# hasindu2008/squigulator

Hardware: AMD Instinct MI355X
Metric: simulated raw samples/sec (higher is better)
Workload: dtype f32+f64

## Files before the change

### squigulator_amd/csrc/h_common.h

```cpp
#pragma once

#if defined(SQG_DEV)
#define SQG_DEV_ENV(name) getenv(name)
#else
#define SQG_DEV_ENV(name) (static_cast<const char*>(nullptr))
#endif
static inline int dev_env_int(const char* v, int dflt) { return v ? atoi(v) : dflt; }

#ifndef SQG_SOURCE_HASH
#define SQG_SOURCE_HASH "unstamped"
#endif
extern "C" const char sqg_source_hash_marker[] = "SQG_SOURCE_HASH=" SQG_SOURCE_HASH ";";
#if defined(SQG_DEV)
static const char kBuildInfo[] = "source_hash=" SQG_SOURCE_HASH ";dev=1";
#else
static const char kBuildInfo[] = "source_hash=" SQG_SOURCE_HASH ";dev=0";
#endif
extern "C" const char* sqg_build_info(void) { return kBuildInfo; }

#include "h_cpus.h"

static uint32_t lcg_pow(uint32_t base, unsigned long long e) {
    uint32_t r = 1, b = base;
    while (e) { if (e & 1) r = lcg_mul(r, b); b = lcg_mul(b, b); e >>= 1; }
// ... 124 lines not shown
    HostPool pool_threads;
    struct DrawAhead* draw_ahead = nullptr;
    sqg_cfg_t cfg;
    int k = 0, num_kmer = 0, T = 0, wlo = 0, whi = 0, nw = 0;
    hipStream_t stream = nullptr;
    uint32_t* d_rows = nullptr;
    float2* d_model = nullptr;
    uint32_t* d_pow = nullptr;
    std::vector<uint32_t> h_pow;
    uint32_t jump2(unsigned long long n) const {
        if (n >> 32) return lcg_pow(lcg_mul(LCG_A, LCG_A), n);
        uint32_t r = h_pow[2 * POW_N + (size_t)(n & (POW_N - 1))];
        const uint32_t hi = (uint32_t)(n >> 10) & (POW_N - 1), hi2 = (uint32_t)(n >> 20);
        if (hi) r = lcg_mul(r, h_pow[3 * POW_N + hi]);
        if (hi2) r = lcg_mul(r, h_pow[4 * POW_N + hi2]);
        return r;
    }
    unsigned int* d_err = nullptr;
    unsigned long long fix_tickets = 0;
    unsigned long long scan_tickets = 0;
    struct Slot {
        int16_t* d_sig = nullptr; size_t sig_cap = 0;
        long long* d_sigoff = nullptr; size_t reads_cap = 0;
        FixEntry* d_fix = nullptr; size_t fix_cap = 0;
        unsigned int* d_fix_count = nullptr;
        FixEntry* d_fix_sh = nullptr; size_t fix_sh_cap = 0;
        unsigned int fix_sh_per = 0;
        unsigned int* d_fix_sh_count = nullptr;
        uint2* d_evrec = nullptr; size_t evrec_cap = 0;
        int* d_slow = nullptr; size_t slow_cap = 0;
        ItemDesc* d_items = nullptr; size_t items_cap = 0;
        uint32_t* d_part = nullptr; size_t part_cap = 0;
        uint32_t* d_lbase = nullptr; size_t lbase_cap = 0;
        int* d_tile_link = nullptr; size_t tile_link_cap = 0;
        uint32_t* d_part_state = nullptr; size_t part_state_cap = 0;
        hipEvent_t cal_a = nullptr, cal_b = nullptr; bool cal_pending = false; long long cal_events = 0; int cal_tries = 0; float cal_ps = 0.f;
        uint2* cal_prev = nullptr; float cal_prev_ps = 0.f;
        unsigned long long gen = 0;
        hipEvent_t done = nullptr;
        hipEvent_t sampled = nullptr;
    } slot[2];
    struct CountSet {
        uint16_t* d_dwell = nullptr; size_t dwell_cap = 0;
        uint32_t* d_tile_so = nullptr; size_t tile_cap = 0;
        unsigned long long* d_seglen = nullptr; size_t seglen_cap = 0;
        size_t seglen_dirty = 0;
        unsigned long long gen = 0;
    } cset[3];
    int num_cu = 256;
    std::deque<sqg_batch*> staged_q;
    hipStream_t fix_stream = nullptr;
    unsigned long long* d_scan_part = nullptr; size_t scan_part_cap = 0;
    uint32_t* d_link_rows = nullptr; size_t link_rows_cap = 0;
    uint32_t* d_pcnt[2] = {nullptr, nullptr}; size_t pcnt_cap[2] = {0, 0};
    uint32_t* d_slice = nullptr; size_t slice_cap = 0;
    uint32_t* d_phist = nullptr; size_t phist_cap = 0;
    double row_bound = 0;
    bool range_mode = false;
    uint32_t* d_xcounts = nullptr; size_t xcounts_cap = 0;
    struct Recycled { uint8_t* d_block; size_t block_bytes; long long* h_sigoff; long long* h_sigoff_dev; size_t h_n; hipEvent_t ev[8];
                      uint8_t* h_meta; size_t h_meta_bytes; hipEvent_t ev_staged; };
    std::vector<Recycled> pool;
    hipStream_t stage_stream = nullptr;
    std::vector<uint32_t> time_c;
    std::vector<long long> off_x, med_x;
    unsigned long long next_stage = 0, next_run = 0, compress_seq = 0;
    unsigned long long runs = 0;
    unsigned int* d_mid_done = nullptr;
    int stage_threads = 0;
    int stage_threads_last = 0;
    int phase_timing_every = 1;
    std::set<unsigned long long> abandoned;
    sqg_timing_t timing = {0, 0, 0, 0, 0, 0, 0, 0};
    bool use_dwell_stream = true, use_kmer_streams = true;
    float delta_x = 0.f;
    float delta_x_measured = 0.f;
    double amp_floor = 0, amp_ceil = 0;
// ... 276 lines not shown
```

### squigulator_amd/csrc/h_context.h

```cpp
#pragma once

extern "C" const char* sqg_strerror(int code) {
    switch (code) {
    case SQG_OK: return "ok";
    case SQG_EINVAL: return "invalid argument or unsupported configuration";
    case SQG_ENOMEM: return "out of memory";
    case SQG_EDEVICE: return "HIP runtime error";
    case SQG_ESEQUENCE: return "batches must be run in staging order";
    case SQG_ENODEVICE: return "no usable HIP device";
    case SQG_EOVERFLOW: return "read too long (>= UINT32_MAX samples) or dwell > 65535";
    case SQG_EIO: return "file I/O error";
    default: return "unknown error";
    }
}

extern "C" const char* sqg_last_error(const sqg_ctx_t* ctx) { return ctx ? ctx->err.c_str() : ""; }

extern "C" int sqg_device_count(void) {
    int n = 0;
    if (hipGetDeviceCount(&n) != hipSuccess) return SQG_ENODEVICE;
    return n;
}

extern "C" int32_t sqg_worker_of(int32_t i, int32_t n_rec, int32_t T) {
    if (T <= 1 || n_rec <= 0) return 0;
    const int32_t step = (n_rec + T - 1) / T;
    return i / step;
}

extern "C" void sqg_destroy(sqg_ctx_t* ctx) {
    if (!ctx) return;
    if (ctx->b5_reader_drain) ctx->b5_reader_drain(ctx->b5_reader, true);
    (void)hipSetDevice(ctx->cfg.device);
    if (ctx->b5_stream) { (void)hipStreamSynchronize(ctx->b5_stream); (void)hipStreamDestroy(ctx->b5_stream); ctx->b5_stream = nullptr; }
    if (ctx->stream) (void)hipStreamSynchronize(ctx->stream);
    if (ctx->fix_stream) (void)hipStreamSynchronize(ctx->fix_stream);
    delete ctx->draw_ahead; ctx->draw_ahead = nullptr;
    (void)hipFree(ctx->d_pcnt[0]); (void)hipFree(ctx->d_pcnt[1]); (void)hipFree(ctx->d_slice); (void)hipFree(ctx->d_phist);
    (void)hipFree(ctx->d_rows); (void)hipFree(ctx->d_link_rows); (void)hipFree(ctx->d_scan_part); (void)hipFree(ctx->d_xcounts); (void)hipFree(ctx->d_model); (void)hipFree(ctx->d_samp_scratch); (void)hipFree(ctx->d_pow); (void)hipFree(ctx->d_err); (void)hipFree(ctx->d_mid_done); if (ctx->h_samp) (void)hipHostFree(ctx->h_samp);
    for (auto& Q : ctx->cset) { (void)hipFree(Q.d_dwell); (void)hipFree(Q.d_tile_so); (void)hipFree(Q.d_seglen); }
    for (auto& S : ctx->slot) {
        (void)hipFree(S.d_sig); (void)hipFree(S.d_sigoff);
        (void)hipFree(S.d_fix); (void)hipFree(S.d_fix_count); (void)hipFree(S.d_fix_sh); (void)hipFree(S.d_fix_sh_count);
        (void)hipFree(S.d_evrec); (void)hipFree(S.d_slow);
        (void)hipFree(S.d_items); (void)hipFree(S.d_part_state); (void)hipFree(S.d_part); (void)hipFree(S.d_lbase); (void)hipFree(S.d_tile_link);
        (void)hipFree(S.cal_prev);
        if (S.cal_a) (void)hipEventDestroy(S.cal_a);
        if (S.cal_b) (void)hipEventDestroy(S.cal_b);
        if (S.done) (void)hipEventDestroy(S.done);
        if (S.sampled) (void)hipEventDestroy(S.sampled);
    }
    (void)hipFree(ctx->d_svb); (void)hipFree(ctx->d_svb_size); (void)hipFree(ctx->d_svb_off);
    (void)hipFree(ctx->d_b5meta); (void)hipFree(ctx->d_b5out); (void)hipFree(ctx->d_b5tab); (void)hipFree(ctx->d_b5size); for (auto* q : ctx->h_b5out) if (q) (void)hipHostFree(q); if (ctx->h_b5meta) (void)hipHostFree(ctx->h_b5meta);
    ctx->chunk.release();
    ctx->site.release();
    ctx->event.release();
    ctx->pileup.release();
    ctx->detect.release();
    ctx->align.release();
    ctx->collapse.release();
    ctx->scale.release();
    (void)hipFree(ctx->d_genome); (void)hipFree(ctx->d_contig_off); (void)hipFree(ctx->d_cum); (void)hipFree(ctx->d_nprefix);
    (void)hipFree(ctx->d_trans_csum); (void)hipFree(ctx->d_trans_idx); (void)hipFree(ctx->d_samp);
    (void)hipFree(ctx->d_meth); (void)hipFree(ctx->d_meth_has); (void)hipFree(ctx->d_meth_st);
    if (ctx->stage_stream) { (void)hipStreamSynchronize(ctx->stage_stream); (void)hipStreamDestroy(ctx->stage_stream); }
    for (auto& r : ctx->pool) { (void)hipFree(r.d_block); (void)hipHostFree(r.h_sigoff); (void)hipHostFree(r.h_meta); for (auto& e : r.ev) if (e) (void)hipEventDestroy(e); if (r.ev_staged) (void)hipEventDestroy(r.ev_staged); }
    ctx->pool.clear();
    if (ctx->fix_stream) (void)hipStreamDestroy(ctx->fix_stream);
    if (ctx->stream) (void)hipStreamDestroy(ctx->stream);
    delete ctx;
}

extern "C" int sqg_create(const sqg_cfg_t* cfg, sqg_ctx_t** out) {
    if (!cfg || !out) return SQG_EINVAL;
    *out = nullptr;
    if (cfg->abi_version != SQG_ABI_VERSION) return SQG_EINVAL;
    if (cfg->kmer_size < 1 || cfg->kmer_size > 9 || !cfg->model) return SQG_EINVAL;
    if (cfg->num_workers < 1 || cfg->worker_lo < 0 || cfg->worker_hi > cfg->num_workers || cfg->worker_lo >= cfg->worker_hi) return SQG_EINVAL;
// ... 162 lines not shown
```

### squigulator_amd/csrc/h_run.h

```cpp
#pragma once

static void count_params(sqg_ctx* c, const sqg_batch* b, sqg_ctx::CountSet& Q, const int n_part, uint32_t* d_pcnt, SigParams& P) {
    const sqg_profile_t& p = c->cfg.profile;
    P.reads = b->d_reads; P.chain_off = b->d_chain_off; P.chain_reads = b->d_chain_reads; P.chain_order = b->d_chain_order; P.bases = b->d_bases;
    P.dwell = c->use_dwell_stream ? Q.d_dwell : nullptr; P.dwell_out = Q.d_dwell; P.seglen_out = Q.d_seglen; P.seglen = Q.d_seglen; P.tile_so = Q.d_tile_so;
    P.dmean = p.dwell_mean; P.dstd = p.dwell_std; P.pw = c->d_pow; P.err = b->d_err; P.delta_x = c->delta_x;
    P.k = c->k; P.num_kmer = c->num_kmer; P.const_sps = (int)p.dwell_mean;
    P.dwell_unbounded = c->dwell_hi > 65535.0 ? 1 : 0;
    P.dwell_pack = c->dwell_hi < 1024.0 ? 1 : 0;
    P.pieces = b->d_pieces; P.piece_total = b->d_piece_total;
    P.pcnt = d_pcnt; P.n_part = n_part; P.n_links = b->n_chains;
}

struct RunStep { const char* name; std::function<int()> go; };
typedef std::vector<RunStep> RunPlan;

struct Run {
    sqg_ctx* c; sqg_batch* b; int phase; const uint32_t* before; const uint32_t* after;
    sqg_ctx::Slot* S; sqg_ctx::Slot* other; sqg_ctx::CountSet* Q;
    int n = 0, n_part = 0, dw = 0;
    bool certified = false, direct = false, fold = false, untimed = false, wave_links = false;
    size_t n_pairs = 0, n_rows = 0;
    unsigned scan_wgs = 0, pgrid = 0;
    uint32_t *d_pcnt = nullptr, *slice_lo = nullptr, *slice_hi = nullptr, *pfirst = nullptr, *pstart = nullptr, *ptotal = nullptr;
    sqg_batch* pre_nb = nullptr;
    SigParams P; ScanArgs SA;
    hipStream_t tail = nullptr;
    bool seglen_zeroed = false;
};

static int run_execute(sqg_ctx* c, const RunPlan& plan) {
    for (const RunStep& st : plan) {
        const int rc = st.go();
        if (rc != SQG_OK) return rc;
        HIPCHK(c, hipGetLastError());
        const int rs = dbg_sync(c, st.name);
        if (rs != SQG_OK) return rs;
    }
    return SQG_OK;
}

static int run_admit(Run& R) {
    sqg_ctx* c = R.c; sqg_batch* b = R.b; const int phase = R.phase;
    if (phase != 2) skip_abandoned(c);
// ... 65 lines not shown
static void run_params(Run& R) {
    sqg_ctx* c = R.c; sqg_batch* b = R.b; const int phase = R.phase, n = R.n;
    sqg_ctx::Slot& S = *R.S; sqg_ctx::CountSet& Q = *R.Q;
    const sqg_profile_t& p = c->cfg.profile;
    R.direct = c->num_kmer <= 4096;
    R.dw = c->use_dwell_stream ? (R.certified && c->dwell_hi < 1.0e6 ? 1 : 2) : 0;
    R.wave_links = b->pieces;
    const int n_part = R.n_part;
    R.d_pcnt = c->d_pcnt[b->run_idx & 1];
    R.pgrid = (unsigned)b->max_slices;
    R.slice_lo = c->d_slice;
    R.slice_hi = R.slice_lo ? R.slice_lo + (size_t)b->max_slices : nullptr;
    R.pfirst = R.slice_hi ? R.slice_hi + (size_t)b->max_slices : nullptr;
    R.pstart = R.pfirst ? R.pfirst + R.n_pairs + 1 : nullptr;
    R.ptotal = R.pstart ? R.pstart + R.n_pairs : nullptr;
    SigParams& P = R.P;
    memset(&P, 0, sizeof P);
    P.link_rows = (b->split && !b->part) ? c->d_link_rows : nullptr;
    P.part = S.d_part; P.part_state = b->part ? S.d_part_state : nullptr;
    P.poff = b->one ? b->d_link_slot : R.d_pcnt ? R.d_pcnt + (size_t)b->n_chains * n_part : nullptr;
    P.link_q = b->d_link_q;
    P.one = b->one ? 1 : 0;
    count_params(c, b, Q, n_part, R.d_pcnt, P);
    P.pstart = R.pstart;
    P.sig_off = S.d_sigoff; P.model = c->d_model; P.rows = c->d_rows;
    P.seed_base = canon((long long)c->cfg.seed + (long long)c->wlo * ((long long)c->num_kmer + 10)); P.seed_step = canon((long long)c->num_kmer + 10);
    P.dig = p.digitisation; P.range = p.range; P.kd = p.digitisation / p.range;
    P.thr_all = c->thr_all;
    P.meth = (c->cfg.flags & SQG_METH) ? 1 : 0; P.num_kmer_pad = n_part * PART_SUB;
    P.meth_top = 1; for (int i = 1; i < c->k; i++) P.meth_top *= 5u;
    P.use_streams = c->use_kmer_streams ? 1 : 0;
    P.rna = (c->cfg.flags & SQG_RNA) ? 1 : 0;
    P.evrec = S.d_evrec;
    if (b->part && b->pieces && !b->one) { P.evrec32 = reinterpret_cast<uint32_t*>(S.d_evrec); P.lbase = S.d_lbase; P.tile_link = S.d_tile_link; }
    P.tile_read = b->d_tile_read; P.stile_read = b->d_stile_read;
    const bool rna_prefix = (c->cfg.flags & SQG_RNA) && (c->cfg.flags & SQG_PREFIX);
    P.shift_len = rna_prefix ? (int)strlen(kAdaptorRna) * (int)p.dwell_mean : 0;
    {
        const double v = 30 * p.digitisation / p.range;
        int32_t t = (v > -2147483649.0 && v < 2147483648.0) ? (int32_t)v : (int32_t)0x80000000u;
        P.shift = (int)(int16_t)(uint16_t)((uint32_t)t & 0xffffu);
    }
    P.slow_count = S.d_fix_count + 1; P.items = S.d_items; P.lean_epl = c->lean_epl;
    P.slow_tiles = (R.certified && c->use_kmer_streams) ? S.d_slow : nullptr;
    R.fold = phase == 0 && n > 0 && b->n_chains > 0 && b->part && !b->one && b->pieces && R.certified && c->use_kmer_streams;
    memset(&R.SA, 0, sizeof R.SA);
    if (n > 0 && phase != 1) {
        ScanArgs& SA = R.SA;
        SA.seglen = Q.d_seglen; SA.n_reads = n; SA.sig_off = S.d_sigoff; SA.host_off = b->h_sigoff_dev; SA.err = b->d_err; SA.counters = S.d_fix_count;
        SA.part = c->d_scan_part; SA.ticket = ++c->scan_tickets; SA.shard_counters = S.d_fix_sh_count;
    }
    if (phase != 2) b->untimed = c->phase_timing_every <= 0 || (b->run_idx % c->phase_timing_every) != 0;
    R.untimed = b->untimed;
}

static void launch_events(Run& R, const int dw, const bool hist) {
    sqg_ctx* c = R.c; sqg_batch* b = R.b; const SigParams& P = R.P;
    constexpr int NT = SQG_EVENT_THREADS, NT_WIDE = 1024;
    const int wide_max = dev_env_int(SQG_DEV_ENV("SQG_EVENTS_WIDE_MAX"), 1200);
    const dim3 g((unsigned)b->n_chains);
    const bool wide = !hist && b->n_chains <= wide_max, direct = R.direct;
#define EVL(N, D, W, H, PT) hipLaunchKernelGGL((k_events<N, D, W, SQG_EVENT_EPT, H, PT>), g, dim3(N), 0, c->stream, P)
#define EVD(N, D, H, PT) do { if (dw == 0) EVL(N, D, 0, H, PT); else if (dw == 1) EVL(N, D, 1, H, PT); else EVL(N, D, 2, H, PT); } while (0)
    if (b->part) { if (hist) EVD(NT, false, true, true); else EVD(NT, false, false, true); }
    else if (wide) { if (direct) EVD(NT_WIDE, true, false, false); else EVD(NT_WIDE, false, false, false); }
    else if (direct) { if (hist) EVD(NT, true, true, false); else EVD(NT, true, false, false); }
    else { if (hist) EVD(NT, false, true, false); else EVD(NT, false, false, false); }
#undef EVD
#undef EVL
}
static void launch_part_events(Run& R, const int dwm, const bool count) {
    sqg_ctx* c = R.c; sqg_batch* b = R.b; const SigParams& P = R.P;
    if (!R.wave_links) { launch_events(R, dwm, count); return; }
    const dim3 g((unsigned)((b->n_chains + PEV_WAVES - 1) / PEV_WAVES)), t(64 * PEV_WAVES);
    if (!count) hipLaunchKernelGGL((k_part_events<0, PEV_SCATTER>), dim3((unsigned)((b->n_chains + PEV_WAVES_SCATTER - 1) / PEV_WAVES_SCATTER)), dim3(64 * PEV_WAVES_SCATTER), 0, c->stream, P, b->n_chains, (uint32_t)b->n_events);
    else if (b->one) {
        if (dwm == 0) hipLaunchKernelGGL((k_part_events<0, PEV_ONE>), g, t, 0, c->stream, P, b->n_chains, (uint32_t)b->n_events);
        else if (dwm == 1) hipLaunchKernelGGL((k_part_events<1, PEV_ONE>), g, t, 0, c->stream, P, b->n_chains, (uint32_t)b->n_events);
        else hipLaunchKernelGGL((k_part_events<2, PEV_ONE>), g, t, 0, c->stream, P, b->n_chains, (uint32_t)b->n_events);
    }
    else if (dwm == 0) hipLaunchKernelGGL((k_part_events<0, PEV_COUNT>), g, t, 0, c->stream, P, b->n_chains, (uint32_t)b->n_events);
    else if (dwm == 1) hipLaunchKernelGGL((k_part_events<1, PEV_COUNT>), g, t, 0, c->stream, P, b->n_chains, (uint32_t)b->n_events);
    else hipLaunchKernelGGL((k_part_events<2, PEV_COUNT>), g, t, 0, c->stream, P, b->n_chains, (uint32_t)b->n_events);
}
#define PLACE_TRIES 3
static int place_calibrate(Run& R) {
    sqg_ctx* c = R.c; sqg_batch* b = R.b; sqg_ctx::Slot& S = *R.S;
    static const bool off = SQG_DEV_ENV("SQG_NO_PLACE") != nullptr;
    if (off || c->cal_runs_left <= 0 || !R.wave_links || !R.P.evrec32 || b->n_events < (1ll << 24)) return SQG_OK;
    if (!S.cal_a) { HIPCHK(c, hipEventCreate(&S.cal_a)); HIPCHK(c, hipEventCreate(&S.cal_b)); }
    if (S.cal_pending) {
        float ms = 0.f;
        HIPCHK(c, hipEventSynchronize(S.cal_b));
        HIPCHK(c, hipEventElapsedTime(&ms, S.cal_a, S.cal_b));
        S.cal_pending = false;
        float ps = ms * 1.0e9f / (float)S.cal_events;
        const char* what = "";
        if (S.cal_prev) {
            if (ps > S.cal_prev_ps) {
                HIPCHK(c, hipEventSynchronize(S.done));
                HIPCHK(c, hipFree(S.d_evrec));
                S.d_evrec = S.cal_prev; ps = S.cal_prev_ps; what = ": slower than the allocation before it, which is taken back";
                R.P.evrec = S.d_evrec; R.P.evrec32 = reinterpret_cast<uint32_t*>(S.d_evrec);
            } else { HIPCHK(c, hipFree(S.cal_prev)); what = ": kept"; }
            S.cal_prev = nullptr;
        }
        S.cal_ps = ps;
        if (getenv("SQG_VERBOSE")) fprintf(stderr, "[sqg] placement: slot %d scatter pass %.0f us = %.3f ps per event%s\n", b->slot, ms * 1.0e3f, ms * 1.0e9f / (float)S.cal_events, what);
        if (S.cal_tries < PLACE_TRIES && c->cal_runs_left >= 3 && S.d_evrec && S.evrec_cap) {
            uint2* fresh = nullptr;
            if (hipMalloc(&fresh, S.evrec_cap * sizeof(uint2)) == hipSuccess) {
                S.cal_prev = S.d_evrec; S.cal_prev_ps = S.cal_ps;
                S.d_evrec = fresh; S.cal_tries++;
                R.P.evrec = S.d_evrec; R.P.evrec32 = reinterpret_cast<uint32_t*>(S.d_evrec);
            } else (void)hipGetLastError();
        }
    }
    c->cal_runs_left--;
    return SQG_OK;
}

static void launch_rows_advance(Run& R) {
    sqg_ctx* c = R.c;
    const dim3 ag((unsigned)((R.n_rows + 255) / 256));
    if (R.direct) hipLaunchKernelGGL(k_rows_advance<true>, ag, dim3(256), 0, c->stream, c->d_rows, c->d_pow, R.n_rows, R.before, c->d_xcounts, R.after);
    else hipLaunchKernelGGL(k_rows_advance<false>, ag, dim3(256), 0, c->stream, c->d_rows, c->d_pow, R.n_rows, R.before, c->d_xcounts, R.after);
}

static void plan_first_pass(Run& R, RunPlan& plan) {
    sqg_ctx* c = R.c; sqg_batch* b = R.b; const int n = R.n;
    if (R.phase == 2) return;
    if (!R.direct && c->use_kmer_streams && n > 0) {
        const double bnd = (double)b->max_wchain_ev * c->dwell_hi;
        if (b->part && !c->range_mode) {
            c->row_bound = std::min((double)LCG_ORD2 + bnd, 4294967295.0) - bnd;
        } else if (c->range_mode || c->row_bound + bnd >= 4294967295.0) {
            plan.push_back({"k_rows_normalize", [&R]() -> int {
                const size_t nrow = (size_t)R.c->nw * (size_t)R.c->num_kmer;
                hipLaunchKernelGGL(k_rows_normalize, dim3((unsigned)((nrow + 255) / 256)), dim3(256), 0, R.c->stream, R.c->d_rows, nrow);
                return SQG_OK; }});
            c->row_bound = (double)LCG_ORD2;
        }
        c->row_bound += bnd;
    }
    if (!R.untimed) plan.push_back({"event: start", [&R]() -> int { HIPCHK(R.c, hipEventRecord(R.b->ev[0], R.c->stream)); return SQG_OK; }});
    if (n > 0 && !c->use_dwell_stream)
        plan.push_back({"upload: constant dwells' totals", [&R]() -> int {
// ... 115 lines not shown
                const dim3 pg((unsigned)((c->num_kmer + 63) / 64), (unsigned)b->n_wchains);
                HIPCHK(c, hipMemsetAsync(c->d_xcounts, 0, R.n_rows * sizeof(uint32_t), c->stream));
                hipLaunchKernelGGL(k_link_totals, pg, dim3(1024), 0, c->stream, R.P, b->d_wlink_off, b->d_wlink_worker, c->d_xcounts);
                return SQG_OK; }});
    }
    if (phase == 1) return;
    plan.push_back({"k_link_prefix", [&R]() -> int {
        sqg_ctx* c = R.c; sqg_batch* b = R.b;
        const dim3 pg((unsigned)((c->num_kmer + 63) / 64), (unsigned)b->n_wchains);
        if (R.direct) hipLaunchKernelGGL(k_link_prefix<true>, pg, dim3(1024), 0, c->stream, R.P, b->d_wlink_off, b->d_wlink_worker, R.before);
        else hipLaunchKernelGGL(k_link_prefix<false>, pg, dim3(1024), 0, c->stream, R.P, b->d_wlink_off, b->d_wlink_worker, R.before);
        return SQG_OK; }});
    if (R.before) plan.push_back({"k_rows_advance", [&R]() -> int { launch_rows_advance(R); return SQG_OK; }});
    plan.push_back({"k_events: the links", [&R]() -> int { launch_events(R, 0, false); return SQG_OK; }});
    (void)c;
}

static void plan_chains(Run& R, RunPlan& plan) {
    if (R.phase == 1) return;
    plan.push_back({"k_events", [&R]() -> int { launch_events(R, R.dw, false); return SQG_OK; }});
}

static int plan_samples(Run& R, RunPlan& plan) {
    sqg_ctx* c = R.c; sqg_batch* b = R.b; const int n = R.n;
    sqg_ctx::Slot& S = *R.S; sqg_ctx::CountSet& Q = *R.Q; SigParams& P = R.P;
    R.tail = c->stream;
    R.seglen_zeroed = false;
    if (n > 0 && b->n_chains > 0) {
        P.sig = S.d_sig; P.fix = S.d_fix; P.fix_count = S.d_fix_count;
        P.fix_sh = S.d_fix_sh; P.fix_sh_cap = S.fix_sh_per; P.fix_sh_count = S.d_fix_sh_count; P.fix_sh_stat = S.d_fix_count + 4; P.host_res = reinterpret_cast<unsigned int*>(b->h_sigoff_dev + (b->h_n - SQG_HRES_LL)); P.fix_tag = (int)(++c->fix_tickets & 0x3fffffffull) + 1;
        P.fix_cap = (unsigned int)std::min<size_t>(S.fix_cap, 0xffffffffu);
        if (b->run_idx < 8 && getenv("SQG_VERBOSE"))
            fprintf(stderr, "[sqg] batch %lld slot %d: sig %p part %p evrec %p part_state %p dwell %p bases %p seglen %p\n", (long long)b->run_idx, b->slot,
                    (void*)S.d_sig, (void*)S.d_part, (void*)S.d_evrec, (void*)S.d_part_state, (void*)Q.d_dwell, (void*)b->d_bases, (void*)Q.d_seglen);
        if (b->run_idx < 8 && getenv("SQG_VERBOSE"))
            fprintf(stderr, "[sqg] batch %lld: %d reads, %lld events, %d links in %d worker chains, %d pieces, %lld slices of %u events at most%s\n", (long long)b->run_idx, n, (long long)b->n_events,
                    b->n_chains, b->n_wchains, b->n_pieces, (long long)b->max_slices, b->slice_len, b->precounted ? "; first event pass: ran ahead, with the previous batch's hand-out" : "");
        if (R.certified && c->use_kmer_streams) {
            if (!R.fold)
                plan.push_back({"k_items", [&R]() -> int { const int ns = (int)R.b->n_stiles; hipLaunchKernelGGL(k_items, dim3((unsigned)((ns + 255) / 256)), dim3(256), 0, R.c->stream, R.P, ns); return SQG_OK; }});
            plan.push_back({"k_samples_lean", [&R]() -> int {
                sqg_ctx* c = R.c; sqg_batch* b = R.b; const SigParams& P = R.P;
                const int n_stiles = (int)b->n_stiles;
                const unsigned lgrid = (unsigned)((n_stiles + 3) / 4);
                if (!R.untimed) HIPCHK(c, hipEventRecord(b->ev[5], c->stream));
#define LEANL(R_, E_) hipLaunchKernelGGL((k_samples_lean<R_, E_>), dim3(lgrid), dim3(256), 0, c->stream, P, n_stiles)
                if (P.rna) { if (c->lean_epl == 4) LEANL(true, 4); else if (c->lean_epl == 2) LEANL(true, 2); else LEANL(true, 1); }
                else { if (c->lean_epl == 4) LEANL(false, 4); else if (c->lean_epl == 2) LEANL(false, 2); else LEANL(false, 1); }
#undef LEANL
                if (!R.untimed) HIPCHK(c, hipEventRecord(b->ev[6], c->stream));
                b->lean_timed = !R.untimed;
                return SQG_OK; }});
            plan.push_back({"k_samples<generic> + k_fixup (their own stream)", [&R]() -> int {
                sqg_ctx* c = R.c; sqg_batch* b = R.b; SigParams& P = R.P;
                HIPCHK(c, hipEventRecord(R.S->sampled, c->stream));
                HIPCHK(c, hipStreamWaitEvent(c->fix_stream, R.S->sampled, 0)); R.tail = c->fix_stream;
                if (SQG_DEV_ENV("SQG_ABL_NOFIX")) return SQG_OK;
                const int n_tiles = (int)b->n_tiles;
                const unsigned sgrid = (unsigned)((n_tiles + 3) / 4);
                hipLaunchKernelGGL((k_samples<1, true>), dim3(std::min(sgrid, 4096u)), dim3(256), 0, R.tail, P, n_tiles);
                P.seglen_zero = 2 * R.n;
                hipLaunchKernelGGL(k_fixup, dim3(FIX_SHARDS), dim3(256), 0, R.tail, P);
                R.seglen_zeroed = true;
                b->fixup_launched = true;
                return SQG_OK; }});
        } else {
            plan.push_back({"k_samples<generic>", [&R]() -> int {
// ... 105 lines not shown
```

### squigulator_amd/csrc/h_stage.h

```cpp
#pragma once

extern "C" void sqg_batch_free(sqg_ctx_t* ctx, sqg_batch_t* b) {
    if (!b) return;
    if (ctx) {
        (void)hipSetDevice(ctx->cfg.device);
        if (b->ran && b->ev[4]) (void)hipEventSynchronize(b->ev[4]);
    }
    if (ctx && b->staged && !b->ran) {
        if ((b->begun || b->precounted) && ctx->stream) (void)hipStreamSynchronize(ctx->stream);
        ctx->abandoned.insert(b->seq);
    }
    if (ctx) for (auto it = ctx->staged_q.begin(); it != ctx->staged_q.end(); ++it) if (*it == b) { ctx->staged_q.erase(it); break; }
    if (ctx && !b->ran && ctx->stage_stream) (void)hipStreamSynchronize(ctx->stage_stream);
    if (b->h_svboff) (void)hipHostFree(b->h_svboff);
    if (ctx && b->d_block && b->h_sigoff && b->ev[0] && ctx->pool.size() < 4) {
        sqg_ctx::Recycled r;
        r.d_block = b->d_block; r.block_bytes = b->block_bytes; r.h_sigoff = b->h_sigoff; r.h_sigoff_dev = b->h_sigoff_dev; r.h_n = b->h_n;
        for (int i = 0; i < 8; i++) r.ev[i] = b->ev[i];
        r.h_meta = b->h_meta; r.h_meta_bytes = b->h_meta_bytes; r.ev_staged = b->ev_staged;
        ctx->pool.push_back(r);
    } else {
        (void)hipFree(b->d_block);
        if (b->h_sigoff) (void)hipHostFree(b->h_sigoff);
        if (b->h_meta) (void)hipHostFree(b->h_meta);
        for (auto& e : b->ev) if (e) (void)hipEventDestroy(e);
        if (b->ev_staged) (void)hipEventDestroy(b->ev_staged);
    }
    delete b;
}

static int grow_cset(sqg_ctx* c, sqg_ctx::CountSet& Q, const sqg_batch* b) {
    int rc2;
    const size_t n = (size_t)b->n;
    if (2 * (n + 1) > Q.seglen_cap) {
        if ((rc2 = ensure(c, (void**)&Q.d_seglen, &Q.seglen_cap, 2 * (n + 1 + n / 2), sizeof(unsigned long long)))) return rc2;
        Q.seglen_dirty = Q.seglen_cap / 2;
    }
    if ((rc2 = ensure(c, (void**)&Q.d_dwell, &Q.dwell_cap, (size_t)b->n_events + 1024, sizeof(uint16_t)))) return rc2;
    if ((rc2 = ensure(c, (void**)&Q.d_tile_so, &Q.tile_cap, (size_t)b->n_tiles + 64, sizeof(uint32_t)))) return rc2;
    return SQG_OK;
}
static int grow_slot(sqg_ctx* c, sqg_ctx::Slot& Z, const sqg_batch* b, bool with_output) {
    int rc2;
    const int n = b->n;
    const bool certified = c->cfg.mode == SQG_MODE_CERTIFIED;
    if ((size_t)n + 1 > Z.reads_cap) {
        HIPCHK(c, hipStreamSynchronize(c->stream));
        (void)hipFree(Z.d_sigoff); Z.d_sigoff = nullptr;
        const size_t cap = (size_t)n + 1 + (size_t)n / 2;
        HIPCHK(c, hipMalloc(&Z.d_sigoff, cap * sizeof(long long)));
        Z.reads_cap = cap;
    }
    if (Z.cal_prev && (size_t)b->n_events + 64 > Z.evrec_cap) {
        HIPCHK(c, hipStreamSynchronize(c->stream)); HIPCHK(c, hipStreamSynchronize(c->fix_stream));
        (void)hipFree(Z.cal_prev); Z.cal_prev = nullptr; Z.cal_pending = false;
    }
    if ((rc2 = ensure(c, (void**)&Z.d_evrec, &Z.evrec_cap, (size_t)b->n_events + 64, sizeof(uint2)))) return rc2;
    if (b->part && (rc2 = ensure(c, (void**)&Z.d_part, &Z.part_cap, (size_t)b->n_events + PART_SLACK, sizeof(uint32_t)))) return rc2;
    if (b->part && b->pieces && !b->one) {
        if ((rc2 = ensure(c, (void**)&Z.d_lbase, &Z.lbase_cap, (size_t)b->n_chains * PART_MAX, sizeof(uint32_t)))) return rc2;
        if ((rc2 = ensure(c, (void**)&Z.d_tile_link, &Z.tile_link_cap, (size_t)b->n_tiles + 64, sizeof(int)))) return rc2;
    }
    if (b->part && (rc2 = ensure(c, (void**)&Z.d_part_state, &Z.part_state_cap, (size_t)b->n_events + PART_SLACK, sizeof(uint32_t)))) return rc2;
    if ((rc2 = ensure(c, (void**)&Z.d_slow, &Z.slow_cap, (size_t)b->n_tiles + 64, sizeof(int)))) return rc2;
    if (certified && c->use_kmer_streams) {
        if ((rc2 = ensure(c, (void**)&Z.d_items, &Z.items_cap, (size_t)b->n_stiles + 64, sizeof(ItemDesc)))) return rc2;
    }
    if (with_output) {
        const double bound = c->dwell_hi * (double)b->n_events;
        if (bound <= 4.0e10) {
            const size_t need = (size_t)bound;
            if ((rc2 = ensure(c, (void**)&Z.d_sig, &Z.sig_cap, need + 64, sizeof(int16_t)))) return rc2;
            if (certified && c->use_kmer_streams)
                if ((rc2 = ensure(c, (void**)&Z.d_fix, &Z.fix_cap, (c->force_fix ? need : need / 256) + 65536, sizeof(FixEntry)))) return rc2;
        }
    }
    return SQG_OK;
}

#include <chrono>
struct Staging {
    sqg_ctx* c; int n; const char* seqs; const int64_t* seq_off; const int32_t* worker; const SampleRec* d_rec; const uint32_t* d_mstate;
    const sqg_profile_t& p;
    const bool rna, prefix;
    const int k;
    sqg_batch* b = nullptr;
    std::vector<ReadDesc> rd; std::vector<int> wk;
    long long nb = 0, nev = 0, ntile = 0, nst = 0;
    int lean_ev = 0;
    std::vector<uint8_t> hb;
    std::vector<int> chain_of, chain_off, chain_reads, wchain_off, wlink_off, wlink_worker;
    int n_wchains = 0, forced = -1;
    std::vector<long long> wchain_ev, chain_ev;
    struct Piece { int read, e_lo, e_hi, pad; };
    std::vector<Piece> pieces;
// ... 479 lines not shown
```

### squigulator_amd/csrc/k_common.h

```cpp
#pragma once

#define LCG_M 2147483647u
#define LCG_A 16807u

#define POW_N 1024
#define POW_TABLES 5
#define POW_TOP 4096
#define POW_WORDS (4 * POW_N + POW_TOP)
#define LCG_ORD2 1073741823u

#define NEAR_ONE_BITS 17

__host__ __device__ static inline uint32_t lcg_mul(uint32_t a, uint32_t b) {
    const unsigned long long p = (unsigned long long)a * b;
    uint32_t r = (uint32_t)(p & LCG_M) + (uint32_t)(p >> 31);
    r = (r & LCG_M) + (r >> 31);
    return r;
}
__device__ static inline uint32_t lcg_mul_lazy(uint32_t a, uint32_t b) {
    const unsigned long long p = (unsigned long long)a * b;
    return (uint32_t)(p & LCG_M) + (uint32_t)(p >> 31);
}

__device__ static inline uint32_t lcg_mul_dbl(uint32_t a, uint32_t b2) {
// ... 105 lines not shown
    int slot0;
};

struct FixEntry {
    long long at;
    long long ev;
    uint32_t c1;
    int read;
    int shifted;
    int pad;
};

struct ItemDesc {
    long long ev_first;
    long long sig_base;
    double offset;
    int n_ev;
    int n_samples;
    uint32_t at0;
    int ev_read0;
    int read;
    int shift_lo, shift_hi;
    int slot_first;
};

struct SigParams {
    const ReadDesc* reads;
    const int* chain_off;
    const int* chain_reads;
    const int* chain_order;
    const uint8_t* bases;
    const uint16_t* dwell;
    uint16_t* dwell_out;
    unsigned long long* seglen_out;
    int seglen_zero;
    double dmean, dstd;
    const unsigned long long* seglen;
    const long long* sig_off;
    const float2* model;
    const uint32_t* pw;
    uint32_t* rows;
    uint32_t* link_rows;
    uint32_t seed_base, seed_step;
    int16_t* sig;
    unsigned int* err;
    FixEntry* fix;
    unsigned int* fix_count;
    unsigned int fix_cap;
    FixEntry* fix_sh;
    unsigned int* fix_sh_count;
    unsigned int fix_sh_cap;
    unsigned int* fix_sh_stat;
    unsigned int* host_res;
    int fix_tag;
    uint2* evrec;
    uint32_t* evrec32;
    uint32_t* lbase;
    int* tile_link;
    uint32_t* tile_so;
    const int* tile_read;
    const int* stile_read;
    ItemDesc* items;
    int lean_epl;
    int* slow_tiles;
    unsigned int* slow_count;
    double dig, range, kd;
// ... 35 lines not shown
```

### squigulator_amd/csrc/k_part_events.h

```cpp
#pragma once

#ifndef PEV_EPL
#define PEV_EPL 8
#endif
#define PEV_SEG (64 * PEV_EPL)
#define PEV_WAVES 4
#ifndef PEV_COUNT_OCC
#define PEV_COUNT_OCC 1
#endif
#define PEV_WAVES_SCATTER 2
#define PEV_HALO 24
#define PEV_WORDS ((PEV_SEG + PEV_HALO) / 16 + 2)

#define PEV_RING 32
#define PEV_LINE 16
#define PEV_TASKS (3 * PART_MAX)
#define PEV_FLUSH_IT 10
template <bool SCATTER>
struct PevWave {
    uint32_t codes[PEV_WORDS];
    uint32_t wslot[PART_MAX];
    uint32_t wbase[SCATTER ? PART_MAX : 1];
    uint32_t flu[SCATTER ? PART_MAX : 1];
    uint32_t ring[SCATTER ? PART_MAX * PEV_RING : 1];
    uint2 tasks[SCATTER ? PEV_TASKS : 1];
};
struct PevTables {
    uint32_t jump[256];
    uint8_t lut[256];
};
template <bool SCATTER>
struct PevLds {
    PevTables t;
    PevWave<SCATTER> w[SCATTER ? PEV_WAVES_SCATTER : PEV_WAVES];
};
__device__ static inline void pev_tables(PevTables& T, const uint32_t* __restrict__ pw, const int tid, const int nthreads) {
    for (int i = tid; i < 256; i += nthreads) { T.jump[i] = pw[2 * POW_N + i] << 1; T.lut[i] = (uint8_t)base_code((uint8_t)i); }
}

__device__ static inline int pev_wave_sum(int v) { return __builtin_amdgcn_readlane(wave_incl_scan_dpp(v), 63); }
__device__ static inline void pev_wave_sum4(int (&v)[4]) {
#define PEV_DPP_STEP(ctrl_, rows_) _Pragma("unroll") for (int i = 0; i < 4; i++) v[i] += __builtin_amdgcn_update_dpp(0, v[i], ctrl_, rows_, 0xf, false);
    PEV_DPP_STEP(0x111, 0xf) PEV_DPP_STEP(0x112, 0xf) PEV_DPP_STEP(0x114, 0xf) PEV_DPP_STEP(0x118, 0xf) PEV_DPP_STEP(0x142, 0xa) PEV_DPP_STEP(0x143, 0xc)
#undef PEV_DPP_STEP
#pragma unroll
    for (int i = 0; i < 4; i++) v[i] = __builtin_amdgcn_readlane(v[i], 63);
}

#define PEV_COUNT 0
#define PEV_SCATTER 1
#define PEV_ONE 2
template <int DW, int MODE>
__device__ static __forceinline__ void pev_link(const SigParams& P, const PevTables& L, PevWave<MODE == PEV_SCATTER>& W, const int li, const uint32_t dump, const int lane) {
    constexpr bool SCATTER = MODE == PEV_SCATTER, ONE = MODE == PEV_ONE;
    static_assert(!SCATTER || DW == 0, "the second pass reads the dwells the first one drew");
    const int chain = P.chain_order[li];
    const int c_lo = P.chain_off[chain], c_hi = P.chain_off[chain + 1];
    const int k = P.k;
    const uint32_t kmask = (1u << (2 * k)) - 1u;
    W.wslot[lane] = (SCATTER && lane < P.n_part) ? P.poff[(size_t)lane * P.n_links + chain] + P.pstart[(size_t)P.link_q[chain] * P.n_part + lane] : 0u;
    uint32_t slot0 = ONE ? P.poff[chain] : 0u;
    if (SCATTER) {
        W.flu[lane] = W.wslot[lane];
        W.wbase[lane] = W.wslot[lane];
        P.lbase[(size_t)chain * PART_MAX + lane] = W.wslot[lane];
    }
    auto flush = [&](const uint32_t a, const uint32_t b) {
        const int nl = b > a ? (int)(((b - 1) >> 4) - (a >> 4)) + 1 : 0;
        const int incl = wave_incl_scan_dpp(nl);
        const int n_task = __builtin_amdgcn_readlane(incl, 63);
        const int at = incl - nl;
#pragma unroll
        for (int i = 0; i < 3; i++) {
            if (i < nl) {
                const uint32_t line = (a >> 4) + (uint32_t)i;
                const uint32_t lo_e = i == 0 ? (a & 15u) : 0u, hi_e = i == nl - 1 ? ((b - 1) & 15u) + 1u : 16u;
                W.tasks[at + i] = make_uint2(line, (uint32_t)lane | lo_e << 8 | hi_e << 16);
            }
        }
        __builtin_amdgcn_wave_barrier();
        asm volatile("" ::: "memory");
        auto put = [&](const int t) {
            const uint2 tk = W.tasks[max(min(t, n_task - 1), 0)];
            const uint32_t e = min(max((uint32_t)lane & 15u, (tk.y >> 8) & 0xffu), (tk.y >> 16) - 1u), sl = tk.x * PEV_LINE + e;
            const uint32_t v = W.ring[(tk.y & (PART_MAX - 1)) * PEV_RING + (sl & (PEV_RING - 1))];
            P.part[n_task > 0 ? sl : dump + (uint32_t)lane] = v;
        };
#pragma unroll
        for (int it = 0; it < PEV_FLUSH_IT; it++) put(4 * it + (lane >> 4));
        for (int t0 = 4 * PEV_FLUSH_IT; t0 < n_task; t0 += 4) put(t0 + (lane >> 4));
        __builtin_amdgcn_wave_barrier();
        asm volatile("" ::: "memory");
    };
    const uint32_t a2seg = DW ? lcg_jump2(P.pw, (uint32_t)PEV_SEG) : 0u, a2half = DW ? lcg_jump2(P.pw, 256u) : 0u;
    const float dw_sf = (float)P.dstd, dw_mf = (float)P.dmean;
    const float dw_eps = P.delta_x * fabsf(dw_sf) + 4.0f * 5.9604645e-8f * (fabsf(dw_mf) + 7.0f * fabsf(dw_sf) + 1.0f) + 1e-6f;

// ... 70 lines not shown
            uint32_t c_blk[PEV_EPL / 4];
            c_blk[0] = c_seg;
#pragma unroll
            for (int h = 1; h < PEV_EPL / 4; h++) c_blk[h] = DW ? (uint32_t)__builtin_amdgcn_readfirstlane((int)lcg_mul(c_blk[h - 1], a2half)) : 0u;
#pragma unroll
            for (int q = 0; q < PEV_EPL; q++) {
                const int j = 64 * q + lane;
                const bool valid = PEV_IN(j);
                if (DW != 0 && valid) {
                    const uint32_t c1 = lcg_mul_dbl(c_blk[q >> 2], L.jump[64 * (q & 3) + lane]);
                    bool decided = false;
                    int v = 0;
                    if (DW == 1) {
                        const float x = box_muller_fast(c1);
                        const float g = __builtin_fmaf(x, dw_sf, dw_mf);
                        const float t = g + LEAN_MAGIC;
                        const float fl = t - LEAN_MAGIC;
                        if (fabsf(g - fl) < 0.5f - dw_eps && c1 <= LCG_M - (1u << NEAR_ONE_BITS)) { v = (int)__float_as_uint(t) - 0x4b400000; decided = true; }
                    }
                    if (!decided) v = dwell_exact(c1, P.dstd, P.dmean);
                    v = max(v, 1 - v);
                    sps[q] = v;
                    P.dwell_out[rd.ev_off + s0 + j] = (uint16_t)v;
                }
            }
            if (DW != 0 && P.dwell_unbounded) {
#pragma unroll
                for (int q = 0; q < PEV_EPL; q++) {
                    if (PEV_IN(64 * q + lane) && sps[q] > 65535) { atomicOr(P.err, 1u); sps[q] = 65535; P.dwell_out[rd.ev_off + s0 + 64 * q + lane] = (uint16_t)65535; }
                }
            }
            if (DW) c_seg = (uint32_t)__builtin_amdgcn_readfirstlane((int)lcg_mul(c_seg, a2seg));
            if (!SCATTER) {
                uint32_t tsum[PEV_EPL];
                if (P.dwell_pack) {
                    static_assert(PEV_EPL == 8, "four packed sums");
                    int two[4];
#pragma unroll
                    for (int h = 0; h < 4; h++) two[h] = (int)((uint32_t)sps[2 * h] | ((uint32_t)sps[2 * h + 1] << 16));
                    pev_wave_sum4(two);
#pragma unroll
                    for (int h = 0; h < 4; h++) { tsum[2 * h] = (uint32_t)two[h] & 0xffffu; tsum[2 * h + 1] = (uint32_t)two[h] >> 16; }
                } else {
#pragma unroll
                    for (int q = 0; q < PEV_EPL; q++) tsum[q] = (uint32_t)pev_wave_sum(sps[q]);
                }
                uint32_t run = 0;
#pragma unroll
                for (int q = 0; q < PEV_EPL; q++) {
                    const int e_q = s0 + 64 * q;
                    if (e_q < ne) {
                        if (lane == 0) P.tile_so[rd.tile_off + (e_q >> 6)] = (uint32_t)done + run;
                        if (rd.ne1 > 0 && rd.ne0 >= e_q && rd.ne0 < e_q + 64)
                            n1 = (long long)done + run + pev_wave_sum(lane < rd.ne0 - e_q ? sps[q] : 0);
                        run += tsum[q];
                        if (ONE) {
                            if (PEV_IN(64 * q + lane)) {
                                const uint32_t sl = slot0 + (uint32_t)(s0 - e_lo + 64 * q + lane);
                                P.part[sl] = rank[q] | ((uint32_t)sps[q] << 16);
                            }
                        } else if (PEV_IN(64 * q + lane)) atomicAdd(&W.wslot[rank[q] >> PART_SUB_BITS], 1u);
                    }
                }
                done += run;
            } else {
                const uint32_t start = W.wslot[lane], flu = W.flu[lane];
                uint32_t slot[PEV_EPL];
                asm volatile("" ::: "memory");
#pragma unroll
                for (int q = 0; q < PEV_EPL; q++) {
                    slot[q] = 0;
                    if (PEV_IN(64 * q + lane)) slot[q] = __hip_atomic_fetch_add(&W.wslot[rank[q] >> PART_SUB_BITS], 1u, __ATOMIC_RELAXED, __HIP_MEMORY_SCOPE_WORKGROUP);
                    asm volatile("" ::: "memory");
                }
                const uint32_t end = W.wslot[lane];
#pragma unroll
                for (int q = 0; q < PEV_EPL; q++) {
                    if (PEV_IN(64 * q + lane))
                        __builtin_nontemporal_store((rank[q] << EVR_REL_BITS) | (slot[q] - W.wbase[rank[q] >> PART_SUB_BITS]), P.evrec32 + rd.ev_off + s0 + 64 * q + lane);
                }
                if (lane < PEV_EPL && s0 + 64 * lane < ne) P.tile_link[rd.tile_off + (s0 >> 6) + lane] = chain;
                if (__builtin_amdgcn_ballot_w64(end - flu > (uint32_t)PEV_RING) == 0ull) {
#pragma unroll
                    for (int q = 0; q < PEV_EPL; q++) {
                        if (PEV_IN(64 * q + lane))
                            W.ring[(rank[q] >> PART_SUB_BITS) * PEV_RING + (slot[q] & (PEV_RING - 1))] = (rank[q] & (PART_SUB - 1)) | ((uint32_t)sps[q] << 16);
                    }
                    const uint32_t upto = max(flu, end & ~(uint32_t)(PEV_LINE - 1));
                    W.flu[lane] = upto;
                    flush(flu, upto);
                } else {
                    flush(flu, start);
                    W.flu[lane] = end;
                    uint2* const sorted = reinterpret_cast<uint2*>(W.ring);
                    uint2* const segbase = W.tasks;
                    const uint32_t cnt = end - start;
                    segbase[lane] = make_uint2(start, (uint32_t)wave_incl_scan_dpp((int)cnt) - cnt);
                    __builtin_amdgcn_wave_barrier();
                    asm volatile("" ::: "memory");
#pragma unroll
                    for (int q = 0; q < PEV_EPL; q++) {
                        if (PEV_IN(64 * q + lane)) {
                            const uint2 sb = segbase[rank[q] >> PART_SUB_BITS];
                            sorted[sb.y + (slot[q] - sb.x)] = make_uint2(slot[q], (rank[q] & (PART_SUB - 1)) | ((uint32_t)sps[q] << 16));
                        }
                    }
                    __builtin_amdgcn_wave_barrier();
                    asm volatile("" ::: "memory");
#pragma unroll
                    for (int q = 0; q < PEV_EPL; q++) {
                        if (PEV_IN(64 * q + lane)) { const uint2 v = sorted[64 * q + lane]; P.part[v.x] = v.y; }
                    }
                    __builtin_amdgcn_wave_barrier();
                    asm volatile("" ::: "memory");
// ... 113 lines not shown
```

Measured before the change: 584.1 billion.

## Move evrec32 and tile_link writes from scatter pass into count pass

The count pass of the partitioned events kernel now takes per-event relative slots with workgroup atomics and writes the packed evrec32 records and tile_link entries itself. The scatter pass no longer stores them. Those buffers move from the per-slot set to the per-count set, so they can be produced ahead by the count pass. The placement calibration now re-allocates the part buffer instead of evrec. This takes stores off the scatter critical path, but the count pass does more work and extra per-countset memory is allocated.

```diff
diff --git a/squigulator_amd/csrc/h_common.h b/squigulator_amd/csrc/h_common.h
--- a/squigulator_amd/csrc/h_common.h
+++ b/squigulator_amd/csrc/h_common.h
@@ -180,10 +180,9 @@
         ItemDesc* d_items = nullptr; size_t items_cap = 0;
         uint32_t* d_part = nullptr; size_t part_cap = 0;
         uint32_t* d_lbase = nullptr; size_t lbase_cap = 0;
-        int* d_tile_link = nullptr; size_t tile_link_cap = 0;
         uint32_t* d_part_state = nullptr; size_t part_state_cap = 0;
         hipEvent_t cal_a = nullptr, cal_b = nullptr; bool cal_pending = false; long long cal_events = 0; int cal_tries = 0; float cal_ps = 0.f;
-        uint2* cal_prev = nullptr; float cal_prev_ps = 0.f;
+        uint32_t* cal_prev = nullptr; float cal_prev_ps = 0.f;
         unsigned long long gen = 0;
         hipEvent_t done = nullptr;
         hipEvent_t sampled = nullptr;
@@ -191,6 +190,8 @@
     struct CountSet {
         uint16_t* d_dwell = nullptr; size_t dwell_cap = 0;
         uint32_t* d_tile_so = nullptr; size_t tile_cap = 0;
+        uint32_t* d_evrec32 = nullptr; size_t evrec32_cap = 0;
+        int* d_tile_link = nullptr; size_t tile_link_cap = 0;
         unsigned long long* d_seglen = nullptr; size_t seglen_cap = 0;
         size_t seglen_dirty = 0;
         unsigned long long gen = 0;
diff --git a/squigulator_amd/csrc/h_context.h b/squigulator_amd/csrc/h_context.h
--- a/squigulator_amd/csrc/h_context.h
+++ b/squigulator_amd/csrc/h_context.h
@@ -38,12 +38,12 @@
     delete ctx->draw_ahead; ctx->draw_ahead = nullptr;
     (void)hipFree(ctx->d_pcnt[0]); (void)hipFree(ctx->d_pcnt[1]); (void)hipFree(ctx->d_slice); (void)hipFree(ctx->d_phist);
     (void)hipFree(ctx->d_rows); (void)hipFree(ctx->d_link_rows); (void)hipFree(ctx->d_scan_part); (void)hipFree(ctx->d_xcounts); (void)hipFree(ctx->d_model); (void)hipFree(ctx->d_samp_scratch); (void)hipFree(ctx->d_pow); (void)hipFree(ctx->d_err); (void)hipFree(ctx->d_mid_done); if (ctx->h_samp) (void)hipHostFree(ctx->h_samp);
-    for (auto& Q : ctx->cset) { (void)hipFree(Q.d_dwell); (void)hipFree(Q.d_tile_so); (void)hipFree(Q.d_seglen); }
+    for (auto& Q : ctx->cset) { (void)hipFree(Q.d_dwell); (void)hipFree(Q.d_tile_so); (void)hipFree(Q.d_seglen); (void)hipFree(Q.d_evrec32); (void)hipFree(Q.d_tile_link); }
     for (auto& S : ctx->slot) {
         (void)hipFree(S.d_sig); (void)hipFree(S.d_sigoff);
         (void)hipFree(S.d_fix); (void)hipFree(S.d_fix_count); (void)hipFree(S.d_fix_sh); (void)hipFree(S.d_fix_sh_count);
         (void)hipFree(S.d_evrec); (void)hipFree(S.d_slow);
-        (void)hipFree(S.d_items); (void)hipFree(S.d_part_state); (void)hipFree(S.d_part); (void)hipFree(S.d_lbase); (void)hipFree(S.d_tile_link);
+        (void)hipFree(S.d_items); (void)hipFree(S.d_part_state); (void)hipFree(S.d_part); (void)hipFree(S.d_lbase);
         (void)hipFree(S.cal_prev);
         if (S.cal_a) (void)hipEventDestroy(S.cal_a);
         if (S.cal_b) (void)hipEventDestroy(S.cal_b);
diff --git a/squigulator_amd/csrc/h_run.h b/squigulator_amd/csrc/h_run.h
--- a/squigulator_amd/csrc/h_run.h
+++ b/squigulator_amd/csrc/h_run.h
@@ -10,6 +10,7 @@
     P.dwell_pack = c->dwell_hi < 1024.0 ? 1 : 0;
     P.pieces = b->d_pieces; P.piece_total = b->d_piece_total;
     P.pcnt = d_pcnt; P.n_part = n_part; P.n_links = b->n_chains;
+    if (b->part && b->pieces && !b->one) { P.evrec32_out = Q.d_evrec32; P.tile_link = Q.d_tile_link; }
 }
 
 struct RunStep { const char* name; std::function<int()> go; };
@@ -141,7 +142,7 @@
     P.use_streams = c->use_kmer_streams ? 1 : 0;
     P.rna = (c->cfg.flags & SQG_RNA) ? 1 : 0;
     P.evrec = S.d_evrec;
-    if (b->part && b->pieces && !b->one) { P.evrec32 = reinterpret_cast<uint32_t*>(S.d_evrec); P.lbase = S.d_lbase; P.tile_link = S.d_tile_link; }
+    if (b->part && b->pieces && !b->one) { P.evrec32 = Q.d_evrec32; P.lbase = S.d_lbase; }
     P.tile_read = b->d_tile_read; P.stile_read = b->d_stile_read;
     const bool rna_prefix = (c->cfg.flags & SQG_RNA) && (c->cfg.flags & SQG_PREFIX);
     P.shift_len = rna_prefix ? (int)strlen(kAdaptorRna) * (int)p.dwell_mean : 0;
@@ -208,20 +209,20 @@
         if (S.cal_prev) {
             if (ps > S.cal_prev_ps) {
                 HIPCHK(c, hipEventSynchronize(S.done));
-                HIPCHK(c, hipFree(S.d_evrec));
-                S.d_evrec = S.cal_prev; ps = S.cal_prev_ps; what = ": slower than the allocation before it, which is taken back";
-                R.P.evrec = S.d_evrec; R.P.evrec32 = reinterpret_cast<uint32_t*>(S.d_evrec);
+                HIPCHK(c, hipFree(S.d_part));
+                S.d_part = S.cal_prev; ps = S.cal_prev_ps; what = ": slower than the allocation before it, which is taken back";
+                R.P.part = S.d_part;
             } else { HIPCHK(c, hipFree(S.cal_prev)); what = ": kept"; }
             S.cal_prev = nullptr;
         }
         S.cal_ps = ps;
         if (getenv("SQG_VERBOSE")) fprintf(stderr, "[sqg] placement: slot %d scatter pass %.0f us = %.3f ps per event%s\n", b->slot, ms * 1.0e3f, ms * 1.0e9f / (float)S.cal_events, what);
-        if (S.cal_tries < PLACE_TRIES && c->cal_runs_left >= 3 && S.d_evrec && S.evrec_cap) {
-            uint2* fresh = nullptr;
-            if (hipMalloc(&fresh, S.evrec_cap * sizeof(uint2)) == hipSuccess) {
-                S.cal_prev = S.d_evrec; S.cal_prev_ps = S.cal_ps;
-                S.d_evrec = fresh; S.cal_tries++;
-                R.P.evrec = S.d_evrec; R.P.evrec32 = reinterpret_cast<uint32_t*>(S.d_evrec);
+        if (S.cal_tries < PLACE_TRIES && c->cal_runs_left >= 3 && S.d_part && S.part_cap) {
+            uint32_t* fresh = nullptr;
+            if (hipMalloc(&fresh, S.part_cap * sizeof(uint32_t)) == hipSuccess) {
+                S.cal_prev = S.d_part; S.cal_prev_ps = S.cal_ps;
+                S.d_part = fresh; S.cal_tries++;
+                R.P.part = S.d_part;
             } else (void)hipGetLastError();
         }
     }
@@ -403,7 +404,7 @@
         P.fix_cap = (unsigned int)std::min<size_t>(S.fix_cap, 0xffffffffu);
         if (b->run_idx < 8 && getenv("SQG_VERBOSE"))
             fprintf(stderr, "[sqg] batch %lld slot %d: sig %p part %p evrec %p part_state %p dwell %p bases %p seglen %p\n", (long long)b->run_idx, b->slot,
-                    (void*)S.d_sig, (void*)S.d_part, (void*)S.d_evrec, (void*)S.d_part_state, (void*)Q.d_dwell, (void*)b->d_bases, (void*)Q.d_seglen);
+                    (void*)S.d_sig, (void*)S.d_part, P.evrec32 ? (void*)P.evrec32 : (void*)S.d_evrec, (void*)S.d_part_state, (void*)Q.d_dwell, (void*)b->d_bases, (void*)Q.d_seglen);
         if (b->run_idx < 8 && getenv("SQG_VERBOSE"))
             fprintf(stderr, "[sqg] batch %lld: %d reads, %lld events, %d links in %d worker chains, %d pieces, %lld slices of %u events at most%s\n", (long long)b->run_idx, n, (long long)b->n_events,
                     b->n_chains, b->n_wchains, b->n_pieces, (long long)b->max_slices, b->slice_len, b->precounted ? "; first event pass: ran ahead, with the previous batch's hand-out" : "");
diff --git a/squigulator_amd/csrc/h_stage.h b/squigulator_amd/csrc/h_stage.h
--- a/squigulator_amd/csrc/h_stage.h
+++ b/squigulator_amd/csrc/h_stage.h
@@ -38,6 +38,10 @@
     }
     if ((rc2 = ensure(c, (void**)&Q.d_dwell, &Q.dwell_cap, (size_t)b->n_events + 1024, sizeof(uint16_t)))) return rc2;
     if ((rc2 = ensure(c, (void**)&Q.d_tile_so, &Q.tile_cap, (size_t)b->n_tiles + 64, sizeof(uint32_t)))) return rc2;
+    if (b->part && b->pieces && !b->one) {
+        if ((rc2 = ensure(c, (void**)&Q.d_evrec32, &Q.evrec32_cap, (size_t)b->n_events + 1024, sizeof(uint32_t)))) return rc2;
+        if ((rc2 = ensure(c, (void**)&Q.d_tile_link, &Q.tile_link_cap, (size_t)b->n_tiles + 64, sizeof(int)))) return rc2;
+    }
     return SQG_OK;
 }
 static int grow_slot(sqg_ctx* c, sqg_ctx::Slot& Z, const sqg_batch* b, bool with_output) {
@@ -51,16 +55,17 @@
         HIPCHK(c, hipMalloc(&Z.d_sigoff, cap * sizeof(long long)));
         Z.reads_cap = cap;
     }
-    if (Z.cal_prev && (size_t)b->n_events + 64 > Z.evrec_cap) {
-        HIPCHK(c, hipStreamSynchronize(c->stream)); HIPCHK(c, hipStreamSynchronize(c->fix_stream));
-        (void)hipFree(Z.cal_prev); Z.cal_prev = nullptr; Z.cal_pending = false;
-    }
-    if ((rc2 = ensure(c, (void**)&Z.d_evrec, &Z.evrec_cap, (size_t)b->n_events + 64, sizeof(uint2)))) return rc2;
+    const bool rec32 = b->part && b->pieces && !b->one;
+    if (b->part && (size_t)b->n_events + PART_SLACK > Z.part_cap) {
+        Z.cal_pending = false;
+        if (Z.cal_prev) {
+            HIPCHK(c, hipStreamSynchronize(c->stream)); HIPCHK(c, hipStreamSynchronize(c->fix_stream));
+            (void)hipFree(Z.cal_prev); Z.cal_prev = nullptr;
+        }
+    }
+    if (!rec32 && (rc2 = ensure(c, (void**)&Z.d_evrec, &Z.evrec_cap, (size_t)b->n_events + 64, sizeof(uint2)))) return rc2;
     if (b->part && (rc2 = ensure(c, (void**)&Z.d_part, &Z.part_cap, (size_t)b->n_events + PART_SLACK, sizeof(uint32_t)))) return rc2;
-    if (b->part && b->pieces && !b->one) {
-        if ((rc2 = ensure(c, (void**)&Z.d_lbase, &Z.lbase_cap, (size_t)b->n_chains * PART_MAX, sizeof(uint32_t)))) return rc2;
-        if ((rc2 = ensure(c, (void**)&Z.d_tile_link, &Z.tile_link_cap, (size_t)b->n_tiles + 64, sizeof(int)))) return rc2;
-    }
+    if (rec32 && (rc2 = ensure(c, (void**)&Z.d_lbase, &Z.lbase_cap, (size_t)b->n_chains * PART_MAX, sizeof(uint32_t)))) return rc2;
     if (b->part && (rc2 = ensure(c, (void**)&Z.d_part_state, &Z.part_state_cap, (size_t)b->n_events + PART_SLACK, sizeof(uint32_t)))) return rc2;
     if ((rc2 = ensure(c, (void**)&Z.d_slow, &Z.slow_cap, (size_t)b->n_tiles + 64, sizeof(int)))) return rc2;
     if (certified && c->use_kmer_streams) {
diff --git a/squigulator_amd/csrc/k_common.h b/squigulator_amd/csrc/k_common.h
--- a/squigulator_amd/csrc/k_common.h
+++ b/squigulator_amd/csrc/k_common.h
@@ -161,6 +161,7 @@
     const uint8_t* bases;
     const uint16_t* dwell;
     uint16_t* dwell_out;
+    uint32_t* evrec32_out;
     unsigned long long* seglen_out;
     int seglen_zero;
     double dmean, dstd;
diff --git a/squigulator_amd/csrc/k_part_events.h b/squigulator_amd/csrc/k_part_events.h
--- a/squigulator_amd/csrc/k_part_events.h
+++ b/squigulator_amd/csrc/k_part_events.h
@@ -20,7 +20,6 @@
 struct PevWave {
     uint32_t codes[PEV_WORDS];
     uint32_t wslot[PART_MAX];
-    uint32_t wbase[SCATTER ? PART_MAX : 1];
     uint32_t flu[SCATTER ? PART_MAX : 1];
     uint32_t ring[SCATTER ? PART_MAX * PEV_RING : 1];
     uint2 tasks[SCATTER ? PEV_TASKS : 1];
@@ -62,7 +61,6 @@
     uint32_t slot0 = ONE ? P.poff[chain] : 0u;
     if (SCATTER) {
         W.flu[lane] = W.wslot[lane];
-        W.wbase[lane] = W.wslot[lane];
         P.lbase[(size_t)chain * PART_MAX + lane] = W.wslot[lane];
     }
     auto flush = [&](const uint32_t a, const uint32_t b) {
@@ -199,6 +197,16 @@
             }
             if (DW) c_seg = (uint32_t)__builtin_amdgcn_readfirstlane((int)lcg_mul(c_seg, a2seg));
             if (!SCATTER) {
+                uint32_t rel[PEV_EPL];
+                if constexpr (MODE == PEV_COUNT) {
+                    asm volatile("" ::: "memory");
+#pragma unroll
+                    for (int q = 0; q < PEV_EPL; q++) {
+                        rel[q] = 0;
+                        if (PEV_IN(64 * q + lane)) rel[q] = __hip_atomic_fetch_add(&W.wslot[rank[q] >> PART_SUB_BITS], 1u, __ATOMIC_RELAXED, __HIP_MEMORY_SCOPE_WORKGROUP);
+                        asm volatile("" ::: "memory");
+                    }
+                }
                 uint32_t tsum[PEV_EPL];
                 if (P.dwell_pack) {
                     static_assert(PEV_EPL == 8, "four packed sums");
@@ -226,10 +234,18 @@
                                 const uint32_t sl = slot0 + (uint32_t)(s0 - e_lo + 64 * q + lane);
                                 P.part[sl] = rank[q] | ((uint32_t)sps[q] << 16);
                             }
-                        } else if (PEV_IN(64 * q + lane)) atomicAdd(&W.wslot[rank[q] >> PART_SUB_BITS], 1u);
+                        }
                     }
                 }
                 done += run;
+                if constexpr (MODE == PEV_COUNT) {
+#pragma unroll
+                    for (int q = 0; q < PEV_EPL; q++) {
+                        if (PEV_IN(64 * q + lane))
+                            __builtin_nontemporal_store((rank[q] << EVR_REL_BITS) | rel[q], P.evrec32_out + rd.ev_off + s0 + 64 * q + lane);
+                    }
+                    if (lane < PEV_EPL && s0 + 64 * lane < ne) P.tile_link[rd.tile_off + (s0 >> 6) + lane] = chain;
+                }
             } else {
                 const uint32_t start = W.wslot[lane], flu = W.flu[lane];
                 uint32_t slot[PEV_EPL];
@@ -241,12 +257,6 @@
                     asm volatile("" ::: "memory");
                 }
                 const uint32_t end = W.wslot[lane];
-#pragma unroll
-                for (int q = 0; q < PEV_EPL; q++) {
-                    if (PEV_IN(64 * q + lane))
-                        __builtin_nontemporal_store((rank[q] << EVR_REL_BITS) | (slot[q] - W.wbase[rank[q] >> PART_SUB_BITS]), P.evrec32 + rd.ev_off + s0 + 64 * q + lane);
-                }
-                if (lane < PEV_EPL && s0 + 64 * lane < ne) P.tile_link[rd.tile_off + (s0 >> 6) + lane] = chain;
                 if (__builtin_amdgcn_ballot_w64(end - flu > (uint32_t)PEV_RING) == 0ull) {
 #pragma unroll
                     for (int q = 0; q < PEV_EPL; q++) {
```

New measurement: 571.5 billion. -2.2%, worse.
